# Pixel-Talk/CanonSwap

Hardware: AMD Instinct MI355X
Metric: frames/sec at 512x512 (generator hot path F->W->T->R->W->G) (higher is better)
Workload: dtype f16; 1 GPU; BASELINE configs[2]: 512x512 video, 64 frames batched per launch on each GPU, steady state over 1280 frames (20 launches per GPU) (256x256 crops in, random-init weights of the real architecture); frames_per_launch_per_gpu=64, frames_total=1280, parallelism=frame-shard x1, identities_resident=1, latency_mode=False, accumulate=fp32, debug_decodes=False

## Files before the change

### canonswap_amd/_isa.py

```python
from __future__ import annotations

import os
import subprocess

from ._build import HALO_NGROUPS, OBJ_DIR


def _disassemble(obj_dir: str, objdump: str, oname: str) -> str:
    obj = os.path.join(obj_dir, oname)
    subprocess.run([objdump, "--offloading", obj], check=True, capture_output=True)
    co = obj + ".0.hipv4-amdgcn-amd-amdhsa--gfx950"
    try:
        return subprocess.run([objdump, "-d", "--no-show-raw-insn", co], check=True, capture_output=True, text=True).stdout
    finally:
        for f in os.listdir(obj_dir):
            if f.startswith(oname + ".0."):
                os.remove(os.path.join(obj_dir, f))


def isa_check(obj_dir: str | None = None) -> dict:
    import re
    obj_dir = obj_dir or OBJ_DIR
    objdump = os.environ.get("LLVM_OBJDUMP", "/opt/rocm/lib/llvm/bin/llvm-objdump")
    if not os.path.exists(objdump):
        raise FileNotFoundError(f"isa_check: {objdump} not found")
    seen = dict(_isa_check_wide(obj_dir, objdump))
    seen.update(_isa_check_lat(obj_dir, objdump))
    for g in range(HALO_NGROUPS):
        txt = _disassemble(obj_dir, objdump, f"conv_halo_g{g}.o")
        for m in re.finditer(r"^[0-9a-f]+ <(_Z16conv_halo_kernelILi\d+ELi\d+ELi(\d+)ELi\d+ELi\d+ELi\d+ELb[01]ELb[01]ELi0EEv10ConvParams)>:\n(.*?)(?=^[0-9a-f]+ <|\Z)",
                             txt, re.S | re.M):
            name, wch, body = m.group(1), int(m.group(2)), m.group(3).split("\n")
            want = f"s_waitcnt vmcnt({3 * wch})"
            kend = max(i for i, l in enumerate(body) if "v_mfma" in l)
            waits = [i for i, l in enumerate(body) if i < kend and l.strip().startswith(want) and "lgkmcnt" not in l]
            if len(waits) < 4:
                raise RuntimeError(f"isa_check: {name}: {len(waits)} x `{want}` in the K loop, expected 4 (one per ring slot)")
            waits = waits[:4]
            loads = [(i, re.search(r"global_load_dwordx4 v\[(\d+):(\d+)\], v\[\d+:\d+\], off", l)) for i, l in enumerate(body)]
            loads = [(i, int(q.group(1))) for i, q in loads if q]
            prime = [r for i, r in loads if i < waits[0]][-4 * wch:]
            if len(prime) != 4 * wch:
                raise RuntimeError(f"isa_check: {name}: the prologue primes {len(prime)} ring registers, expected {4 * wch}")
            for k, w in enumerate(waits):
                slot = prime[k * wch:(k + 1) * wch]
                end = waits[k + 1] if k + 1 < 4 else len(body)
                seg = body[w:end]
                rel = [i for i, r in loads if w < i < end and r in slot]
                if len(rel) < wch:
                    raise RuntimeError(f"isa_check: {name}: ring slot {k} is not reloaded into v{slot} after its wait")
                first_reload = min(rel) - w
                uses = [j for j, l in enumerate(seg[:first_reload]) if "v_mfma" in l and any(f"v[{r}:{r + 3}]" in l for r in slot)]
                if not uses:
                    raise RuntimeError(f"isa_check: {name}: no MFMA reads ring slot {k} (v{slot}) between its wait and its reload")
            tail = "\n".join(body[waits[-1]:])
            if "s_waitcnt vmcnt(0)" not in tail:
                raise RuntimeError(f"isa_check: {name}: the ring is not drained (s_waitcnt vmcnt(0)) before the epilogue")
            seen[name] = len(waits)
    if not seen:
        raise RuntimeError("isa_check: no dynamic-shape conv_halo kernel found in the objects (name mangling changed?)")
    return seen


def _isa_check_lat(obj_dir: str, objdump: str) -> dict:
    import re
    txt = _disassemble(obj_dir, objdump, "conv_lat.o")
    seen = {}
    for m in re.finditer(r"^[0-9a-f]+ <(\S*conv_lat_kernel\S*)>:\n(.*?)(?=^[0-9a-f]+ <|\Z)", txt, re.S | re.M):
        name, body = m.group(1), [l.split("//")[0].strip() for l in m.group(2).split("\n")]
        body = [l for l in body if l]
        mf = [i for i, l in enumerate(body) if l.startswith("v_mfma")]
        if not mf:
            raise RuntimeError(f"isa_check: {name}: no MFMA")
        if any(l.startswith(("s_cbranch", "s_branch")) for l in body[mf[0]:mf[-1]]):
            raise RuntimeError(f"isa_check: {name}: a branch inside the K loop (the walk assumes straight-line code)")
        for i, l in enumerate(body):
            if re.search(r"\bm0\b", l):
                ok = l.startswith("s_mov_b32 m0,") and any(b.startswith("buffer_load") and b.endswith("lds") for b in body[i + 1:i + 3])
                if not ok:
                    raise RuntimeError(f"isa_check: {name}: `{l}` touches m0 outside the hidden LDS-DMA sequence")
        nvm, open_dma, nbar, ndma = 0, [], 0, 0
        for i, l in enumerate(body[:mf[-1] + 1]):
            op = l.split()[0]
            if op.startswith(("global_load", "buffer_load", "global_store", "buffer_store", "scratch_load", "scratch_store")):
                if op.startswith("buffer_load") and l.endswith("lds"):
                    open_dma.append(nvm); ndma += 1
                nvm += 1
            if op == "s_barrier":
                nbar += 1
                w = next((body[j] for j in range(i - 1, max(i - 6, -1), -1) if body[j].startswith("s_waitcnt") and "vmcnt" in body[j]), None)
                if w is None and not open_dma:
                    continue
                if w is None:
                    raise RuntimeError(f"isa_check: {name}: barrier {nbar} of the K loop has no vmcnt wait in front of it")
                n = int(re.search(r"vmcnt\((\d+)\)", w).group(1))
                for idx in open_dma:
                    if nvm - idx - 1 < n:
                        raise RuntimeError(f"isa_check: {name}: `{w}` before barrier {nbar} does not cover a DMA piece issued {nvm - idx - 1} vector-memory instructions earlier")
                open_dma = []
        if open_dma:
            raise RuntimeError(f"isa_check: {name}: {len(open_dma)} DMA pieces are never waited for at a chunk head")
        if len(mf) not in (8 * 6 * 8, 8 * 6 * 16) or ndma != 24:
            raise RuntimeError(f"isa_check: {name}: {len(mf)} MFMAs / {ndma} DMA instructions, expected 384 or 768 / 24")
        seen[name] = len(mf)
    if not seen:
        raise RuntimeError("isa_check: no conv_lat kernel found in conv_lat.o (name mangling changed?)")
    return seen


def _isa_check_wide(obj_dir: str, objdump: str) -> dict:
    seen = _isa_check_ring(obj_dir, objdump, "conv_wide.o", r"\S*conv_wide_kernel\S*", 18 * 64)
    seen.update(_isa_check_ring(obj_dir, objdump, "conv_halo_g1.o", r"_Z16conv_halo_kernelILi32ELi8ELi5ELi2ELi2ELi0ELb1ELb0ELi[789]E\S*", None))
    return seen


def _isa_check_ring(obj_dir: str, objdump: str, oname: str, name_re: str, expect_mfma) -> dict:
    import re
    txt = _disassemble(obj_dir, objdump, oname)
    seen = {}
    for m in re.finditer(r"^[0-9a-f]+ <(" + name_re + r")>:\n(.*?)(?=^[0-9a-f]+ <|\Z)", txt, re.S | re.M):
        name, body = m.group(1), m.group(2).split("\n")
        writer, waited, issued, nmfma = {}, {}, {}, 0
        pending, nvm = [], 0
        mf = [i for i, l in enumerate(body) if "v_mfma" in l]
        lo, hi = (mf[0], mf[-1]) if mf else (0, 0)
        for li, l in enumerate(body):
            t = l.split("//")[0].strip()
            if not t:
                continue
            op = t.split()[0]
            if op.startswith("s_waitcnt") and "vmcnt" in t:
                n = int(re.search(r"vmcnt\((\d+)\)", t).group(1))
                for r in waited:
                    if nvm - issued.get(r, -1) - 1 >= n:
                        waited[r] = True
                pending = [q for q in pending if nvm - q[1] - 1 < n]
            if op.startswith(("s_cbranch", "s_branch", "s_endpgm")) or li < lo:
                pending = []
            if pending and not op.startswith(("s_", "global_store", "buffer_store", "ds_write", "scratch_store")):
                mm0 = re.match(r"\S+\s+(v\[(\d+):(\d+)\]|v(\d+))", t)
                if mm0 and not (op.startswith("buffer_load") and t.endswith("lds")):
                    dst = set(range(int(mm0.group(2)), int(mm0.group(3)) + 1)) if mm0.group(2) else {int(mm0.group(4))}
                    for regs, _ in pending:
                        if regs & dst:
                            raise RuntimeError(f"isa_check: {name}: `{t}` writes v{sorted(regs & dst)} while an untracked ring load into them is in flight")
            if op.startswith(("global_load", "buffer_load", "global_store", "buffer_store", "scratch_load", "scratch_store", "global_atomic")):
                if op.startswith("global_load_dwordx4") and li >= lo:
                    q = re.match(r"\S+\s+v\[(\d+):(\d+)\]", t)
                    if q:
                        pending.append((set(range(int(q.group(1)), int(q.group(2)) + 1)), nvm))
                nvm += 1
            if op.startswith("v_mfma"):
                ops = re.findall(r"([av])\[(\d+):(\d+)\]", t)
                if len(ops) < 4 or ops[1][0] != "v":
                    raise RuntimeError(f"isa_check: {name}: MFMA with a weight operand outside the VGPRs: {t}")
                nmfma += 1
                for r in range(int(ops[1][1]), int(ops[1][2]) + 1):
                    if not writer.get(r, "").startswith("global_load_dwordx4"):
                        raise RuntimeError(f"isa_check: {name}: v{r}, a weight operand of `{t}`, was last written by `{writer.get(r)}` (a copy of a ring register?)")
                    if not waited.get(r, False):
                        raise RuntimeError(f"isa_check: {name}: no vmcnt wait between the ring load of v{r} and `{t}`")
                continue
            if op.startswith(("global_store", "buffer_store", "ds_write", "scratch_store", "s_", "buffer_load_dwordx4")) and "lds" in t + " lds" and not op.startswith("global_load"):
                if not op.startswith(("v_", "ds_read", "global_load", "scratch_load")):
                    continue
            mm = re.match(r"\S+\s+(v\[(\d+):(\d+)\]|v(\d+))", t)
            if mm and not op.startswith(("global_store", "buffer_store", "ds_write", "scratch_store")) and not (op.startswith("buffer_load") and t.endswith("lds")):
                rng = range(int(mm.group(2)), int(mm.group(3)) + 1) if mm.group(2) else [int(mm.group(4))]
                is_vm = op.startswith(("global_load", "buffer_load", "scratch_load"))
                for r in rng:
                    writer[r] = op
                    waited[r] = False
                    issued[r] = (nvm - 1) if is_vm else -1
        if expect_mfma is not None and nmfma != expect_mfma:
            raise RuntimeError(f"isa_check: {name}: {nmfma} MFMAs in the kernel, expected {expect_mfma}")
        seen[name] = nmfma
    if not seen:
        raise RuntimeError(f"isa_check: no kernel matching {name_re} found in {oname} (name mangling changed?)")
    return seen
```

### canonswap_amd/csrc/vol32.hip

```cpp
#include "conv_epilogue.h"

namespace {

constexpr int V_TW = 8;
constexpr int V_NC = V_TW + 2;
constexpr int V_CS = 17 * 16;
constexpr int V_RS = V_NC * V_CS;
constexpr int V_WLO = 27 * 2 * 1024;
constexpr int V_SROWS = 8;
enum { V_EPI_F16 = 0,
       V_EPI_RES = 1,
       V_EPI_STAT = 2 };

template <bool SPLIT, int EPI = 0> struct VRing {
    static constexpr int K = SPLIT ? 2 : 4;
    static constexpr int RING = K + 2;
    static constexpr int QS = ((RING * V_RS + 16 + 255) / 256) * 256;
    static constexpr int IMG = 4 * QS;
    static constexpr int NIMG = SPLIT ? 2 : 1;
    static constexpr int AUX = NIMG * IMG;
    static constexpr int RROWS = K + 1;
    static constexpr int RSLOT = 4 * 4096;
    static constexpr int lds(int epi) { return AUX + (SPLIT ? V_WLO : 0) + (epi == 1 ? RROWS * RSLOT : 0); }
};

struct Vol32Params {
    const half_t* in; const half_t* zero;
    int in_sN, in_sH, in_sW;
    int N, H, W;
    const half_t* wgt;
    const float* bias;
    float sl0, sl1;
    const float* res; int res_sN, res_sH, res_sW;
    void* out0; int o0_sN, o0_sH, o0_sW;
    half_t* out1; int o1_sN, o1_sH, o1_sW;
    const float* s2; const float* t2;
    float* stat_out; int stat_nblk;
    int srows;
    const float* xf_y; int xy_sN, xy_sH, xy_sW;
    const float* xf_res; int xr_sN, xr_sH, xr_sW;
    float* xf_out; int xo_sN, xo_sH, xo_sW;
    const float* xf_stats; const float* xf_gamma; const float* xf_beta; float xf_slope;
    int nstrips, nseg, seg_rows, items;
#ifdef V32_TL
    unsigned long long* tl; long tl_cap;
#endif
};

typedef unsigned int u4v __attribute__((ext_vector_type(4)));

#ifdef V32_TL
#define TLS(i) do { __builtin_amdgcn_sched_barrier(0); const unsigned long long t_ = __builtin_amdgcn_s_memtime(); tl_acc[i] += t_ - tl_last; tl_last = t_; \
                    __builtin_amdgcn_sched_barrier(0); } while (0)
#else
#define TLS(i) do { } while (0)
#endif

template <int N> __device__ __forceinline__ void wait_vm() { asm volatile("s_waitcnt vmcnt(%0)" ::"n"(N) : "memory"); }

template <int EPI, bool SPLIT, int XF>
__global__ void __launch_bounds__(256, 1) vol32_kernel(const Vol32Params p)
{
    static_assert(XF == 0 || (SPLIT && EPI == V_EPI_STAT), "transform staging exists for the split-precision statistics kernel");
    extern __shared__ __attribute__((aligned(16))) unsigned char smem[];
    using R = VRing<SPLIT, EPI>;
    constexpr int K = R::K, RING = R::RING, QS = R::QS, IMG = R::IMG, NIMG = R::NIMG;
    constexpr int VOX = SPLIT ? 64 : 32;
    static_assert(!(SPLIT && EPI == V_EPI_RES), "the residual ring and the W_lo fragments share the LDS region after the images");
    constexpr int ND = XF ? 0 : 3 * NIMG + (EPI == V_EPI_RES ? 4 : 0), NR = 0, NS = EPI == V_EPI_F16 ? 2 : (EPI == V_EPI_RES ? 6 : 4);
    constexpr int NW0 = NR + (K - 2) * (ND + NR + NS), NW = NW0 + NS;
    static_assert(NW <= 63, "vmcnt is a 6-bit counter");
    const int tid = threadIdx.x, lane = tid & 63;
    const int wave = __builtin_amdgcn_readfirstlane(tid >> 6);
    const int l15 = lane & 15, l4 = lane >> 4;
#ifdef V32_TL
    unsigned long long tl_acc[10] = {0, 0, 0, 0, 0, 0, 0, 0, 0, 0}, tl_last = __builtin_amdgcn_s_memtime();
#endif

    for (int i = tid * 16; i < NIMG * IMG; i += 256 * 16) *(u4v*)(smem + i) = (u4v){0u, 0u, 0u, 0u};
    h8_t wr[27][2];
    {
        const half_t* wl = p.wgt + ep_lane_row(1, l15) * 32 + l4 * 8;
#pragma unroll
        for (int t = 0; t < 27; ++t) {
            wr[t][0] = *(const h8_t*)(wl + t * 1024 + ep_frag_row(1, 0) * 32);
            wr[t][1] = *(const h8_t*)(wl + t * 1024 + ep_frag_row(1, 1) * 32);
        }
        if constexpr (SPLIT) {
            for (int f = wave; f < 54; f += 4) {
                const h8_t v = *(const h8_t*)(wl + (27 + (f >> 1)) * 1024 + ep_frag_row(1, f & 1) * 32);
                *(h8_t*)(smem + R::AUX + f * 1024 + lane * 16) = v;
            }
        }
    }
    float bias_v[8], s2_v[8], t2_v[8];
#pragma unroll
    for (int r = 0; r < 8; ++r) {
        bias_v[r] = p.bias ? p.bias[l4 * 8 + r] : 0.f;
        s2_v[r] = p.s2 ? p.s2[l4 * 8 + r] : 1.f;
        t2_v[r] = p.s2 ? p.t2[l4 * 8 + r] : 0.f;
    }
    __syncthreads();

    int s_off[3]; bool s_on[3];
#pragma unroll
    for (int j = 0; j < 3; ++j) {
        const int idx = j * 64 + lane, col = idx / 17, ds = idx % 17;
        s_on[j] = idx < V_NC * 17 && ds != 0;
        s_off[j] = col * p.in_sW + (ds - 1) * VOX + wave * 8;
    }
    const int lanebase = l4 * QS + l15 * 16 + (2 * wave) * V_CS;
    const unsigned lane_el = (unsigned)(l15 * 32 + l4 * 8);
    const unsigned char* wlo = smem + R::AUX + lane * 16;

    const int G = (int)gridDim.x;
    int u = (int)blockIdx.x;
    if ((G & 7) == 0) u = (u & 7) * (G >> 3) + (u >> 3);

    for (int item = u; item < p.items; item += G) {
        int t = item;
        const int strip = t % p.nstrips; t /= p.nstrips;
        const int seg = t % p.nseg;
        const int n = t / p.nseg;
        const int w0 = strip * V_TW;
        const int h0 = seg * p.seg_rows, h1 = (h0 + p.seg_rows < p.H) ? h0 + p.seg_rows : p.H;
        bool c_ok[3];
#pragma unroll
        for (int j = 0; j < 3; ++j) {
            const int col = (j * 64 + lane) / 17;
            c_ok[j] = s_on[j] && (unsigned)(w0 - 1 + col) < (unsigned)p.W;
        }
        const half_t* in_n = p.in + (long)n * p.in_sN + (long)(w0 - 1) * p.in_sW;
        const unsigned nb_o0 = (unsigned)(n * p.o0_sN + (w0 + 2 * wave) * p.o0_sW);
        const unsigned nb_o1 = (unsigned)(n * p.o1_sN + (w0 + 2 * wave) * p.o1_sW);
        const unsigned nb_rs = (unsigned)(n * p.res_sN + (w0 + 2 * wave) * p.res_sW);
        auto stage_piece = [&](int r, int slot, int rslot, int q) {
            if (q < 3 * NIMG) {
                const int im = q / 3, j = q % 3;
                const bool rok = (unsigned)r < (unsigned)p.H && r <= h1;
                const half_t* rp = in_n + (long)r * p.in_sH;
                unsigned char* dst = smem + wave * QS + slot * V_RS;
                if (s_on[j]) {
                    const half_t* src = (rok && c_ok[j]) ? rp + s_off[j] + im * 32 : p.zero;
                    __builtin_amdgcn_global_load_lds((const __attribute__((address_space(1))) void*)src,
                                                     (__attribute__((address_space(3))) void*)(dst + im * IMG + j * 1024), 16, 0, 0);
                }
            } else if constexpr (EPI == V_EPI_RES) {
                const int j = q - 3 * NIMG;
                const int rc = (unsigned)r < (unsigned)p.H ? r : 0;
                const float* rsrc = p.res + (nb_rs + (unsigned)(rc * p.res_sH) + lane_el);
                unsigned char* rdst = smem + R::AUX + rslot * R::RSLOT + wave * 4096;
                __builtin_amdgcn_global_load_lds((const __attribute__((address_space(1))) void*)(rsrc + (j >> 1) * p.res_sW + (j & 1) * 4),
                                                 (__attribute__((address_space(3))) void*)(rdst + j * 1024), 16, 0, 0);
            }
        };
        auto stage_row = [&](int r, int slot, int rslot) {
#pragma unroll
            for (int q = 0; q < ND; ++q) stage_piece(r, slot, rslot, q);
        };
        constexpr bool XRES = XF >= 2 && ((XF - 2) & 1) != 0, XWB = XF >= 2 && ((XF - 2) & 2) != 0;
        float4 xr[XF ? 3 : 1][2], xs[XRES ? 3 : 1][2];
        float xsc[XF >= 2 ? 8 : 1], xsh[XF >= 2 ? 8 : 1];
        const int xq = tid & 3;
        if constexpr (XF >= 2) {
#pragma unroll
            for (int r = 0; r < 8; ++r) {
                const int c = xq * 8 + r;
                const float mean = p.xf_stats[((long)n * 32 + c) * 2], rstd = p.xf_stats[((long)n * 32 + c) * 2 + 1];
                xsc[r] = gn_scale(rstd, p.xf_gamma[c]);
                xsh[r] = gn_shift(mean, xsc[r], p.xf_beta[c]);
            }
        }
        int xoff[XF ? 3 : 1]; bool xcok[XF ? 3 : 1];
        if constexpr (XF != 0) {
#pragma unroll
            for (int it = 0; it < 3; ++it) {
                int idx = it * 256 + tid;
                if (idx >= V_NC * 64) idx -= 128;
                const int col = idx >> 6, d = (idx >> 2) & 15;
                xoff[it] = n * p.xy_sN + (w0 - 1 + col) * p.xy_sW + d * 32 + xq * 8;
                xcok[it] = (unsigned)(w0 - 1 + col) < (unsigned)p.W;
            }
        }
        const unsigned xsafe = (unsigned)(n * p.xy_sN + w0 * p.xy_sW + h0 * p.xy_sH + ((tid >> 2) & 15) * 32 + xq * 8);
        auto xf_load_to = [&](int r, int it, float4 (&dr)[2], float4 (&ds)[2]) {
            if constexpr (XF != 0) {
                const bool okl = xcok[it] && (unsigned)r < (unsigned)p.H && r <= h1;
                const unsigned o = okl ? (unsigned)(xoff[it] + r * p.xy_sH) : xsafe;
                const float* y = p.xf_y + o;
                dr[0] = *(const float4*)y; dr[1] = *(const float4*)(y + 4);
                if constexpr (XRES) {
                    const float* x = p.xf_res + o;
                    ds[0] = *(const float4*)x; ds[1] = *(const float4*)(x + 4);
                }
            }
        };
        auto xf_load = [&](int r, int it) { xf_load_to(r, it, xr[it], xs[XRES ? it : 0]); };
        float xa[8];
        auto xf_write_from = [&](int r, int slot, int it, int part, const float4 (&xr)[2], const float4 (&xs)[2]) {
            if constexpr (XF != 0) {
                int idx = it * 256 + tid;
                if (idx >= V_NC * 64) idx -= 128;
                const bool ok = xcok[it] && (unsigned)r < (unsigned)p.H && r <= h1;
#pragma unroll
                for (int k = 0; k < 8; ++k) {
                    if (part >= 0 && (k >> 2) != part) continue;
                    const float v = ((const float*)&xr[k >> 2])[k & 3];
                    if constexpr (XRES) xa[k] = gn_lrelu(v, xsc[k], xsh[k], ((const float*)&xs[k >> 2])[k & 3], p.xf_slope);
                    else if constexpr (XF >= 2) xa[k] = gn_lrelu(v, xsc[k], xsh[k], 0.f, p.xf_slope);
                    else xa[k] = v;
                    if (!ok) xa[k] = 0.f;
                }
                if (part >= 0 && part != 2) return;
                h8_t hi, lo;
#pragma unroll
                for (int k = 0; k < 8; ++k) { hi[k] = (half_t)xa[k]; lo[k] = (half_t)(xa[k] - (float)hi[k]); }
                unsigned char* dst = smem + xq * QS + (idx >> 6) * V_CS + (((idx >> 2) & 15) + 1) * 16 + slot * V_RS;
                *(h8_t*)dst = hi; *(h8_t*)(dst + IMG) = lo;
                if constexpr (XWB) {
                    float* o = ok ? p.xf_out + (unsigned)(xoff[it] + r * p.xy_sH) : (float*)p.zero;
                    *(float4*)o = make_float4(xa[0], xa[1], xa[2], xa[3]); *(float4*)(o + 4) = make_float4(xa[4], xa[5], xa[6], xa[7]);
                }
            }
        };
        auto xf_write = [&](int r, int slot, int it, int part) { xf_write_from(r, slot, it, part, xr[it], xs[XRES ? it : 0]); };
        if constexpr (XF != 0) {
            float4 pr[3][3][2], ps[XRES ? 3 : 1][3][2];
#pragma unroll
            for (int i = 0; i < 3; ++i)
#pragma unroll
                for (int it = 0; it < 3; ++it) xf_load_to(h0 - 1 + i, it, pr[i][it], ps[XRES ? i : 0][it]);
#pragma unroll
            for (int i = 0; i < 3; ++i)
#pragma unroll
                for (int it = 0; it < 3; ++it) xf_write_from(h0 - 1 + i, i, it, -1, pr[i][it], ps[XRES ? i : 0][it]);
        } else {
#pragma unroll
            for (int i = 0; i <= K; ++i) stage_row(h0 - 1 + i, i, i == 0 ? K : i - 1);
        }
        TLS(0);
        __syncthreads();
        TLS(1);

        float ov[2][8]; h8_t ou[2];
        bool have = false;
        int hprev = 0;
        auto store_piece = [&](int k) {
            constexpr int PC = NS / 2;
            const int c = k / PC, w = k % PC;
            const unsigned o = nb_o0 + (unsigned)(hprev * p.o0_sH + c * p.o0_sW) + lane_el;
            if constexpr (EPI != V_EPI_F16) {
                if (w == 0) *(float4*)((float*)p.out0 + o) = make_float4(ov[c][0], ov[c][1], ov[c][2], ov[c][3]);
                if (w == 1) *(float4*)((float*)p.out0 + o + 4) = make_float4(ov[c][4], ov[c][5], ov[c][6], ov[c][7]);
                if constexpr (EPI == V_EPI_RES) {
                    if (w == 2) *(h8_t*)(p.out1 + (nb_o1 + (unsigned)(hprev * p.o1_sH + c * p.o1_sW) + lane_el)) = ou[c];
                }
            } else {
                h8_t x;
#pragma unroll
                for (int r = 0; r < 8; ++r) x[r] = ep_h(ov[c][r]);
                *(h8_t*)((half_t*)p.out0 + o) = x;
            }
        };
        auto flush = [&]() {
#pragma unroll
            for (int k = 0; k < NS; ++k) store_piece(k);
        };
        float st_s[8], st_q[8];
#pragma unroll
        for (int r = 0; r < 8; ++r) { st_s[r] = 0.f; st_q[r] = 0.f; }

        int s0 = 0, r0 = 0;
        for (int h = h0; h < h1; ++h) {
            int sk = s0 + K + 1; sk -= sk >= RING ? RING : 0;
            int rk = r0 + K; rk -= rk >= R::RROWS ? R::RROWS : 0;
            f4_t rr[2][2];
            if constexpr (EPI == V_EPI_RES) {
#pragma unroll
                for (int c = 0; c < 2; ++c)
#pragma unroll
                    for (int i = 0; i < 2; ++i) rr[c][i] = *(const f4_t*)(wlo + r0 * R::RSLOT + wave * 4096 + (c * 2 + i) * 1024);
            }
            int rb[3];
#pragma unroll
            for (int kh = 0; kh < 3; ++kh) { int sl = s0 + kh; sl -= sl >= RING ? RING : 0; rb[kh] = lanebase + sl * V_RS; }
            f4_t acc[2][2];
#pragma unroll
            for (int c = 0; c < 2; ++c)
#pragma unroll
                for (int ci = 0; ci < 2; ++ci) acc[c][ci] = (f4_t){0.f, 0.f, 0.f, 0.f};
            constexpr int NG = SPLIT ? 27 : 9;
            constexpr int XL0 = 4, XW0 = 17;
            h8_t fa[4], fb[4];
            h8_t wa[SPLIT ? 3 : 1][2], wb[SPLIT ? 3 : 1][2];
            auto rd = [&](h8_t (&f)[4], h8_t (&wl2)[SPLIT ? 3 : 1][2], int G2) {
                const int pass = G2 / 9, g = G2 % 9, kd = g / 3, kh = g % 3;
                const int img = (SPLIT && pass == 2) ? IMG : 0;
#pragma unroll
                for (int i = 0; i < 4; ++i) f[i] = *(const h8_t*)(smem + rb[kh] + img + i * V_CS + kd * 16);
                if constexpr (SPLIT) {
                    if (pass == 1) {
#pragma unroll
                        for (int kw = 0; kw < 3; ++kw)
#pragma unroll
                            for (int ci = 0; ci < 2; ++ci) wl2[kw][ci] = *(const h8_t*)(wlo + ((g * 3 + kw) * 2 + ci) * 1024);
                    }
                }
            };
            rd(fa, wa, 0);
#pragma unroll
            for (int G2 = 0; G2 < NG; ++G2) {
                h8_t (&cur)[4] = (G2 & 1) ? fb : fa;
                h8_t (&wcur)[SPLIT ? 3 : 1][2] = (G2 & 1) ? wb : wa;
                h8_t (&wnxt)[SPLIT ? 3 : 1][2] = (G2 & 1) ? wa : wb;
                if constexpr (XF != 0) { if (G2 >= XW0 && G2 < XW0 + 9) xf_write(h + 2, sk, (G2 - XW0) / 3, (G2 - XW0) % 3); }
                if (G2 + 1 < NG) {
                    h8_t (&nxt)[4] = (G2 & 1) ? fa : fb;
                    rd(nxt, wnxt, G2 + 1);
                }
                const int pass = G2 / 9, g = G2 % 9;
#pragma unroll
                for (int kw = 0; kw < 3; ++kw)
#pragma unroll
                    for (int c = 0; c < 2; ++c)
#pragma unroll
                        for (int ci = 0; ci < 2; ++ci) {
                            const h8_t a = (SPLIT && pass == 1) ? wcur[SPLIT ? kw : 0][ci] : wr[g * 3 + kw][ci];
                            acc[c][ci] = __builtin_amdgcn_mfma_f32_16x16x32_f16(a, cur[kw + c], acc[c][ci], 0, 0, 0);
                        }
                if (G2 + 1 < NG) {
                    const int nrd = 4 + ((SPLIT && (G2 + 1) / 9 == 1) ? 6 : 0);
                    const bool conv_here = XF != 0 && G2 >= XW0 && G2 < XW0 + 9;
#pragma unroll
                    for (int i = 0; i < 11; ++i) {
                        __builtin_amdgcn_sched_group_barrier(0x008, 1, 0);
                        if (i < nrd) __builtin_amdgcn_sched_group_barrier(0x100, 1, 0);
                        if (conv_here) __builtin_amdgcn_sched_group_barrier(0x002, 4, 0);
                    }
                }
                __builtin_amdgcn_sched_barrier(0);
                if constexpr (XF == 0) {
                    constexpr int NM = ND + NS;
#pragma unroll
                    for (int m = G2 * NM / NG; m < (G2 + 1) * NM / NG; ++m) {
                        asm volatile("" ::: "memory");
                        if (m < ND) stage_piece(h + K, sk, rk, m);
                        else if (have) store_piece(m - ND);
                        asm volatile("" ::: "memory");
                    }
                    __builtin_amdgcn_sched_barrier(0);
                } else {
                    if (G2 < NS && have) store_piece(G2);
                    if (G2 >= XL0 && G2 < XL0 + 6 && ((G2 - XL0) & 1) == 0) xf_load(h + 2, (G2 - XL0) >> 1);
                    __builtin_amdgcn_sched_barrier(0);
                }
            }
            TLS(4);
#pragma unroll
            for (int c = 0; c < 2; ++c) {
#pragma unroll
                for (int r = 0; r < 8; ++r) {
                    float v = acc[c][r >> 2][r & 3] + bias_v[r];
                    v = lin_act(v, p.sl0);
                    if constexpr (EPI == V_EPI_RES) v += rr[c][r >> 2][r & 3];
                    ov[c][r] = v;
                    if constexpr (EPI == V_EPI_STAT) { st_s[r] += v; st_q[r] = fmaf(v, v, st_q[r]); }
                    if constexpr (EPI == V_EPI_RES) {
                        const float a = v * s2_v[r] + t2_v[r];
                        ou[c][r] = ep_h(lin_act(a, p.sl1));
                    }
                }
            }
            if constexpr (EPI == V_EPI_STAT) {
                if (((h + 1) % p.srows) == 0 || h + 1 == h1) {
                    const int blk = (h / p.srows) * (p.W / 2) + (w0 / 2 + wave);
                    float pa[8], pb[8];
#pragma unroll
                    for (int r = 0; r < 8; ++r) {
                        float a = st_s[r], b = st_q[r];
                        st_s[r] = 0.f; st_q[r] = 0.f;
#pragma unroll
                        for (int o = 1; o < 16; o <<= 1) { a += __shfl_xor(a, o, 64); b += __shfl_xor(b, o, 64); }
                        pa[r] = a; pb[r] = b;
                    }
                    if (l15 == 0) {
                        float4* dst = (float4*)(p.stat_out + (((long)n * p.stat_nblk + blk) * 32 + l4 * 8) * 2);
#pragma unroll
                        for (int r = 0; r < 4; ++r) dst[r] = make_float4(pa[2 * r], pb[2 * r], pa[2 * r + 1], pb[2 * r + 1]);
                    }
                }
            }
            have = true; hprev = h;
            s0 = s0 + 1 == RING ? 0 : s0 + 1;
            r0 = r0 + 1 == R::RROWS ? 0 : r0 + 1;
            TLS(5);
            if constexpr (XF != 0) asm volatile("s_waitcnt lgkmcnt(0)" ::: "memory");
            else if (h > h0 + K - 2) wait_vm<NW>();
            else wait_vm<NW0>();
            TLS(6);
            __builtin_amdgcn_s_barrier();
            asm volatile("" ::: "memory");
            TLS(7);
#ifdef V32_TL
            tl_acc[9] += 1;
#endif
        }
        if (have) flush();
        __syncthreads();
        TLS(8);
    }
#ifdef V32_TL
    if (p.tl && lane == 0) {
        const long wi = (long)blockIdx.x * 4 + wave;
        if (wi < p.tl_cap) {
            unsigned hwid;
            asm volatile("s_getreg_b32 %0, hwreg(HW_REG_HW_ID)" : "=s"(hwid));
            unsigned long long* o = p.tl + wi * 12;
#pragma unroll
            for (int i = 0; i < 10; ++i) o[i] = tl_acc[i];
            o[10] = hwid; o[11] = __builtin_amdgcn_s_memrealtime();
        }
    }
#endif
}

int g_ncu = 0;
#ifdef V32_TL
unsigned long long* g_v32_tl = nullptr;
long g_v32_cap = 0;
#endif

}

#ifdef V32_TL
extern "C" void cs_debug_set_vol32_tl(void* buf, long cap) { g_v32_tl = (unsigned long long*)buf; g_v32_cap = cap; }
#endif

bool vol32_supported(const ConvParams& p)
{
    if (p.KD != 3 || p.KH != 3 || p.KW != 3 || p.Cout_pad != 32 || p.Cout != 32 || p.D != 16 || p.inD != 16 || (p.W % V_TW) != 0) return false;
    if (p.xf_kind) {
        if (!p.hilo || p.Cin != 96 || !p.stat_out || (p.xf_kind != 1 && p.xf_kind != 2) || !p.xf_y.p || p.xf_y.sD != 32) return false;
        if (p.xf_kind == 2 && (!p.xf_stats || !p.xf_gamma || !p.xf_beta)) return false;
        if (p.xf_res.p && (p.xf_kind != 2 || p.xf_res.sD != 32)) return false;
        if (p.xf_out.p && (p.xf_kind != 2 || p.xf_out.sD != 32)) return false;
    } else if (p.hilo ? (p.Cin != 96 || p.in_sD != 64) : (p.Cin != 32 || p.in_sD != 32)) return false;
    if (p.up_shift || p.cg || p.wslot || p.sk_out || p.ragged || p.pixscale || p.stats || p.pool_hw || p.spmul) return false;
    if (p.act0 > ACT_LRELU || p.act1 > ACT_LRELU) return false;
    if (p.res.p && (!p.res_f32 || p.res.sD != 32)) return false;
    if (p.out0.p && p.out0.sD != 32) return false;
    if (p.out1.p && p.out1.sD != 32) return false;
    if (!p.out0.p) return false;
    if (p.hilo && !p.stat_out) return false;
    if (p.stat_out) return p.out0_f32 && !p.res.p && !p.out1.p;
    if (p.res.p) return p.out0_f32 && p.out1.p && !p.hilo;
    return !p.out0_f32 && !p.out1.p;
}

static int vol32_srows(const ConvParams& p) { return p.v32_srows > 0 ? p.v32_srows : V_SROWS; }
int vol32_stat_nblk(const ConvParams& p) { const int sr = vol32_srows(p); return ((p.H + sr - 1) / sr) * (p.W / 2); }

int launch_vol32(const ConvParams& p, hipStream_t st)
{
    if (!vol32_supported(p)) { cs_set_error("vol32: not a 3x3x3 32 -> 32 convolution on a [N][H][W][16][32] volume this kernel supports"); return -1; }
    if (ep_check_extents(p, "vol32")) return -1;
    const long in_span = (long)(p.N - 1) * p.in_sN + (long)(p.H - 1) * p.in_sH + (long)(p.W - 1) * p.in_sW + 1024;
    if (!p.xf_kind && in_span >= (1L << 31)) { cs_set_error("vol32: the input spans 2^31 elements or more"); return -1; }
    if (!g_ncu) {
        int dev = 0, n = 0;
        if (hipGetDevice(&dev) != hipSuccess || hipDeviceGetAttribute(&n, hipDeviceAttributeMultiprocessorCount, dev) != hipSuccess || n < 1) n = 256;
        g_ncu = n;
    }
    Vol32Params k;
    k.in = p.in; k.zero = p.zero; k.in_sN = (int)p.in_sN; k.in_sH = (int)p.in_sH; k.in_sW = (int)p.in_sW;
    k.N = p.N; k.H = p.H; k.W = p.W;
    k.wgt = p.wgt; k.bias = p.bias;
    k.sl0 = p.act0 == ACT_NONE ? 1.f : (p.act0 == ACT_LRELU ? p.slope0 : 0.f);
    k.sl1 = p.act1 == ACT_NONE ? 1.f : (p.act1 == ACT_LRELU ? p.slope1 : 0.f);
    k.res = (const float*)p.res.p; k.res_sN = (int)p.res.sN; k.res_sH = (int)p.res.sH; k.res_sW = (int)p.res.sW;
    k.out0 = p.out0.p; k.o0_sN = (int)p.out0.sN; k.o0_sH = (int)p.out0.sH; k.o0_sW = (int)p.out0.sW;
    k.out1 = (half_t*)p.out1.p; k.o1_sN = (int)p.out1.sN; k.o1_sH = (int)p.out1.sH; k.o1_sW = (int)p.out1.sW;
    k.s2 = p.s2; k.t2 = p.t2;
    k.stat_out = p.stat_out; k.stat_nblk = vol32_stat_nblk(p); k.srows = vol32_srows(p);
    k.xf_y = (const float*)p.xf_y.p; k.xy_sN = (int)p.xf_y.sN; k.xy_sH = (int)p.xf_y.sH; k.xy_sW = (int)p.xf_y.sW;
    k.xf_res = (const float*)p.xf_res.p; k.xr_sN = (int)p.xf_res.sN; k.xr_sH = (int)p.xf_res.sH; k.xr_sW = (int)p.xf_res.sW;
    k.xf_out = (float*)p.xf_out.p; k.xo_sN = (int)p.xf_out.sN; k.xo_sH = (int)p.xf_out.sH; k.xo_sW = (int)p.xf_out.sW;
    k.xf_stats = p.xf_stats; k.xf_gamma = p.xf_gamma; k.xf_beta = p.xf_beta; k.xf_slope = p.xf_slope;
    if (p.xf_kind) {
        auto same = [&](const TDesc& t) { return !t.p || (t.sN == p.xf_y.sN && t.sH == p.xf_y.sH && t.sW == p.xf_y.sW); };
        if (!same(p.xf_res) || !same(p.xf_out)) { cs_set_error("vol32: the transform-staging volumes must share their strides"); return -1; }
        const long lim = 1L << 31;
        auto span = [&](const TDesc& t) { return (long)(p.N - 1) * t.sN + (long)(p.H - 1) * t.sH + (long)(p.W - 1) * t.sW + 512; };
        if (span(p.xf_y) >= lim || (p.xf_res.p && span(p.xf_res) >= lim) || (p.xf_out.p && span(p.xf_out) >= lim)) {
            cs_set_error("vol32: a transform-staging tensor spans 2^31 elements or more"); return -1;
        }
    }
#ifdef V32_TL
    k.tl = g_v32_tl; k.tl_cap = g_v32_cap;
#endif
    k.nstrips = p.W / V_TW;
    int nseg = 1;
    while ((long)p.N * k.nstrips * nseg < g_ncu && (p.H % (nseg * 2 * k.srows)) == 0) nseg *= 2;
    k.seg_rows = (p.H + nseg - 1) / nseg;
    k.nseg = (p.H + k.seg_rows - 1) / k.seg_rows;
    k.items = p.N * k.nstrips * k.nseg;
    int grid = k.items < g_ncu ? k.items : g_ncu;
    if (grid >= 8) grid &= ~7;
    const bool split = p.hilo != 0;
    const int epi = p.stat_out ? V_EPI_STAT : (p.res.p ? V_EPI_RES : V_EPI_F16);
    auto go = [&](auto kern, size_t lds) -> int {
        if (lds > 64 * 1024) {
            hipError_t e = hipFuncSetAttribute((const void*)kern, hipFuncAttributeMaxDynamicSharedMemorySize, (int)lds);
            if (e != hipSuccess) { cs_set_error("vol32: opting into %zu bytes of LDS failed: %s", lds, hipGetErrorString(e)); return -1; }
        }
        hipLaunchKernelGGL(kern, dim3((unsigned)grid), dim3(256), lds, st, k);
        return 0;
    };
    int r = -1;
    if (split) {
        if (epi != V_EPI_STAT) { cs_set_error("vol32: the split-precision kernel exists with the statistics epilogue only"); return -1; }
        if (p.xf_kind == 2) {
            const int v = (p.xf_res.p ? 1 : 0) | (p.xf_out.p ? 2 : 0);
            if (v == 0) r = go(vol32_kernel<V_EPI_STAT, true, 2>, VRing<true, V_EPI_STAT>::lds(V_EPI_STAT));
            else if (v == 1) r = go(vol32_kernel<V_EPI_STAT, true, 3>, VRing<true, V_EPI_STAT>::lds(V_EPI_STAT));
            else if (v == 2) r = go(vol32_kernel<V_EPI_STAT, true, 4>, VRing<true, V_EPI_STAT>::lds(V_EPI_STAT));
            else r = go(vol32_kernel<V_EPI_STAT, true, 5>, VRing<true, V_EPI_STAT>::lds(V_EPI_STAT));
        }
        else if (p.xf_kind == 1) r = go(vol32_kernel<V_EPI_STAT, true, 1>, VRing<true, V_EPI_STAT>::lds(V_EPI_STAT));
        else r = go(vol32_kernel<V_EPI_STAT, true, 0>, VRing<true, V_EPI_STAT>::lds(V_EPI_STAT));
    } else {
        if (epi == V_EPI_STAT) r = go(vol32_kernel<V_EPI_STAT, false, 0>, VRing<false, V_EPI_STAT>::lds(V_EPI_STAT));
        else if (epi == V_EPI_RES) r = go(vol32_kernel<V_EPI_RES, false, 0>, VRing<false, V_EPI_RES>::lds(V_EPI_RES));
        else r = go(vol32_kernel<V_EPI_F16, false, 0>, VRing<false, V_EPI_F16>::lds(V_EPI_F16));
    }
    if (r) return r;
    hipError_t e = hipGetLastError();
    if (e != hipSuccess) { cs_set_error("vol32 launch: %s", hipGetErrorString(e)); return -1; }
    return 0;
}
```

Measured before the change: 536.3 frames/s.

## Add eight-wave vol32 kernel splitting output channels across wave pairs

Adds a 512-thread variant of the split-precision vol32 3D conv kernel for the transform-staging cases. Each pair of waves splits the 32 output channels into two 16-channel fragments, so a wave holds only its half of the weights in registers. The staging loads and transforms for row h+2 are interleaved into the MFMA loop with sched_group_barriers. It is on by default behind an env var and is verified by a new ISA check for MFMA count, no scratch or AGPR use, and correct waitcnt placement. The trade-off is more waves per block at launch bounds of one block per CU, with the intent of better latency hiding, at the cost of more barrier participants.

```diff
diff --git a/canonswap_amd/_isa.py b/canonswap_amd/_isa.py
--- a/canonswap_amd/_isa.py
+++ b/canonswap_amd/_isa.py
@@ -26,6 +26,7 @@
         raise FileNotFoundError(f"isa_check: {objdump} not found")
     seen = dict(_isa_check_wide(obj_dir, objdump))
     seen.update(_isa_check_lat(obj_dir, objdump))
+    seen.update(_isa_check_vol32_w8(obj_dir, objdump))
     for g in range(HALO_NGROUPS):
         txt = _disassemble(obj_dir, objdump, f"conv_halo_g{g}.o")
         for m in re.finditer(r"^[0-9a-f]+ <(_Z16conv_halo_kernelILi\d+ELi\d+ELi(\d+)ELi\d+ELi\d+ELi\d+ELb[01]ELb[01]ELi0EEv10ConvParams)>:\n(.*?)(?=^[0-9a-f]+ <|\Z)",
@@ -105,6 +106,42 @@
         seen[name] = len(mf)
     if not seen:
         raise RuntimeError("isa_check: no conv_lat kernel found in conv_lat.o (name mangling changed?)")
+    return seen
+
+
+def _isa_check_vol32_w8(obj_dir: str, objdump: str) -> dict:
+    import re
+    txt = _disassemble(obj_dir, objdump, "vol32.o")
+    seen = {}
+    for m in re.finditer(r"^[0-9a-f]+ <(\S*vol32_w8_kernelILi(\d)E\S*)>:\n(.*?)(?=^[0-9a-f]+ <|\Z)", txt, re.S | re.M):
+        name, body = m.group(1), [l.split("//")[0].strip() for l in m.group(3).split("\n")]
+        body = [l for l in body if l]
+        mf = [i for i, l in enumerate(body) if l.startswith("v_mfma")]
+        if len(mf) != 162:
+            raise RuntimeError(f"isa_check: {name}: {len(mf)} MFMAs, expected 162")
+        top = max((i for i, l in enumerate(body[:mf[0]]) if l == "s_barrier"), default=0)
+        since = None
+        for l in body[top:mf[-1] + 1]:
+            op = l.split()[0]
+            if op.startswith("global_load"):
+                since = 0
+            elif op.startswith(("global_store", "global_atomic")) and since is not None:
+                since += 1
+            elif op == "s_waitcnt" and "vmcnt" in l:
+                n = int(re.search(r"vmcnt\((\d+)\)", l).group(1))
+                if since is None or n < since:
+                    raise RuntimeError(f"isa_check: {name}: `{l}` in the K loop waits for more than the staging loads in front of it "
+                                       "(a load result carried over the back-edge?)")
+        for l in body:
+            if l.startswith("scratch_") or re.search(r"\ba(\d+|\[\d+:\d+\])", l):
+                raise RuntimeError(f"isa_check: {name}: `{l}`: scratch or AGPRs in a kernel with a 256-register budget")
+        tail = body[mf[-1]:]
+        bar = next((i for i, l in enumerate(tail) if l == "s_barrier"), None)
+        if bar is None or not any(l.startswith("s_waitcnt") and "lgkmcnt(0)" in l for l in tail[max(bar - 4, 0):bar]):
+            raise RuntimeError(f"isa_check: {name}: no `s_waitcnt lgkmcnt(0)` in front of the step's barrier")
+        seen[name] = len(mf)
+    if sorted(int(re.search(r"vol32_w8_kernelILi(\d)E", k).group(1)) for k in seen) != [1, 2, 3, 5]:
+        raise RuntimeError(f"isa_check: vol32.o holds the eight-wave instantiations {sorted(seen)}, expected XF 1, 2, 3, 5")
     return seen
 
 
diff --git a/canonswap_amd/csrc/vol32.hip b/canonswap_amd/csrc/vol32.hip
--- a/canonswap_amd/csrc/vol32.hip
+++ b/canonswap_amd/csrc/vol32.hip
@@ -412,6 +412,254 @@
 #ifdef V32_TL
     if (p.tl && lane == 0) {
         const long wi = (long)blockIdx.x * 4 + wave;
+        if (wi < p.tl_cap) {
+            unsigned hwid;
+            asm volatile("s_getreg_b32 %0, hwreg(HW_REG_HW_ID)" : "=s"(hwid));
+            unsigned long long* o = p.tl + wi * 12;
+#pragma unroll
+            for (int i = 0; i < 10; ++i) o[i] = tl_acc[i];
+            o[10] = hwid; o[11] = __builtin_amdgcn_s_memrealtime();
+        }
+    }
+#endif
+}
+
+template <int XF>
+__global__ void __launch_bounds__(512, 1) vol32_w8_kernel(const Vol32Params p)
+{
+    static_assert(XF >= 1 && XF <= 5, "the eight-wave form exists for the transform-staging variants");
+    extern __shared__ __attribute__((aligned(16))) unsigned char smem[];
+    using R = VRing<true, V_EPI_STAT>;
+    constexpr int K = R::K, RING = R::RING, QS = R::QS, IMG = R::IMG;
+    static_assert(K == 2, "row h + 2 is fetched, transformed and written within step h");
+    constexpr int NS = 2;
+    constexpr int NP = V_NC * 128;
+    const int tid = threadIdx.x, lane = tid & 63;
+    const int wave = __builtin_amdgcn_readfirstlane(tid >> 6);
+    const int cp = wave & 3, fr = wave >> 2;
+    const int l15 = lane & 15, l4 = lane >> 4;
+#ifdef V32_TL
+    unsigned long long tl_acc[10] = {0, 0, 0, 0, 0, 0, 0, 0, 0, 0}, tl_last = __builtin_amdgcn_s_memtime();
+#endif
+
+    for (int i = tid * 16; i < 2 * IMG; i += 512 * 16) *(u4v*)(smem + i) = (u4v){0u, 0u, 0u, 0u};
+    h8_t wr[27];
+    {
+        const half_t* wl = p.wgt + (fr * 16 + l15) * 32 + l4 * 8;
+#pragma unroll
+        for (int t = 0; t < 27; ++t) wr[t] = *(const h8_t*)(wl + t * 1024);
+        for (int t = cp; t < 27; t += 4) {
+            const h8_t v = *(const h8_t*)(wl + (27 + t) * 1024);
+            *(h8_t*)(smem + R::AUX + (t * 2 + fr) * 1024 + lane * 16) = v;
+        }
+    }
+    float bias_v[4];
+#pragma unroll
+    for (int r = 0; r < 4; ++r) bias_v[r] = p.bias ? p.bias[fr * 16 + l4 * 4 + r] : 0.f;
+    __syncthreads();
+
+    const int lanebase = l4 * QS + l15 * 16 + (2 * cp) * V_CS;
+    const unsigned lane_el = (unsigned)(l15 * 32 + fr * 16 + l4 * 4);
+    const unsigned char* wlo = smem + R::AUX + fr * 1024 + lane * 16;
+
+    const int G = (int)gridDim.x;
+    int u = (int)blockIdx.x;
+    if ((G & 7) == 0) u = (u & 7) * (G >> 3) + (u >> 3);
+
+    for (int item = u; item < p.items; item += G) {
+        int t = item;
+        const int strip = t % p.nstrips; t /= p.nstrips;
+        const int seg = t % p.nseg;
+        const int n = t / p.nseg;
+        const int w0 = strip * V_TW;
+        const int h0 = seg * p.seg_rows, h1 = (h0 + p.seg_rows < p.H) ? h0 + p.seg_rows : p.H;
+        const unsigned nb_o0 = (unsigned)(n * p.o0_sN + (w0 + 2 * cp) * p.o0_sW);
+        constexpr bool XRES = XF >= 2 && ((XF - 2) & 1) != 0, XWB = XF >= 2 && ((XF - 2) & 2) != 0;
+        float4 xr[3], xs[XRES ? 3 : 1];
+        float xsc[XF >= 2 ? 4 : 1], xsh[XF >= 2 ? 4 : 1];
+        const int xc = tid & 7;
+        if constexpr (XF >= 2) {
+#pragma unroll
+            for (int r = 0; r < 4; ++r) {
+                const int c = xc * 4 + r;
+                const float mean = p.xf_stats[((long)n * 32 + c) * 2], rstd = p.xf_stats[((long)n * 32 + c) * 2 + 1];
+                xsc[r] = gn_scale(rstd, p.xf_gamma[c]);
+                xsh[r] = gn_shift(mean, xsc[r], p.xf_beta[c]);
+            }
+        }
+        auto xf_idx = [&](int it) { const int idx = it * 512 + tid; return idx >= NP ? idx - 256 : idx; };
+        int xoff[3]; bool xcok[3];
+#pragma unroll
+        for (int it = 0; it < 3; ++it) {
+            const int idx = xf_idx(it), col = idx >> 7, d = (idx >> 3) & 15;
+            xoff[it] = n * p.xy_sN + (w0 - 1 + col) * p.xy_sW + d * 32 + xc * 4;
+            xcok[it] = (unsigned)(w0 - 1 + col) < (unsigned)p.W;
+        }
+        const unsigned xsafe = (unsigned)(n * p.xy_sN + w0 * p.xy_sW + h0 * p.xy_sH + ((tid >> 3) & 15) * 32 + xc * 4);
+        auto xf_load_to = [&](int r, int it, float4& dr, float4& ds) {
+            const bool okl = xcok[it] && (unsigned)r < (unsigned)p.H && r <= h1;
+            const unsigned o = okl ? (unsigned)(xoff[it] + r * p.xy_sH) : xsafe;
+            dr = *(const float4*)(p.xf_y + o);
+            if constexpr (XRES) ds = *(const float4*)(p.xf_res + o);
+        };
+        auto xf_load = [&](int r, int it) { xf_load_to(r, it, xr[it], xs[XRES ? it : 0]); };
+        float xa[4];
+        auto xf_write_from = [&](int r, int slot, int it, int part, const float4& yr, const float4& sr) {
+            const int idx = xf_idx(it);
+            const bool ok = xcok[it] && (unsigned)r < (unsigned)p.H && r <= h1;
+            if (part <= 0) {
+#pragma unroll
+                for (int k = 0; k < 4; ++k) {
+                    const float v = ((const float*)&yr)[k];
+                    if constexpr (XRES) xa[k] = gn_lrelu(v, xsc[k], xsh[k], ((const float*)&sr)[k], p.xf_slope);
+                    else if constexpr (XF >= 2) xa[k] = gn_lrelu(v, xsc[k], xsh[k], 0.f, p.xf_slope);
+                    else xa[k] = v;
+                    if (!ok) xa[k] = 0.f;
+                }
+            }
+            if (part == 0) return;
+            h4_t hi, lo;
+#pragma unroll
+            for (int k = 0; k < 4; ++k) { hi[k] = (half_t)xa[k]; lo[k] = (half_t)(xa[k] - (float)hi[k]); }
+            unsigned char* dst = smem + (xc >> 1) * QS + (idx >> 7) * V_CS + (((idx >> 3) & 15) + 1) * 16 + (xc & 1) * 8 + slot * V_RS;
+            *(h4_t*)dst = hi; *(h4_t*)(dst + IMG) = lo;
+            if constexpr (XWB) {
+                float* o = ok ? p.xf_out + (unsigned)(xoff[it] + r * p.xy_sH) : (float*)p.zero;
+                *(float4*)o = make_float4(xa[0], xa[1], xa[2], xa[3]);
+            }
+        };
+        auto xf_write = [&](int r, int slot, int it, int part) { xf_write_from(r, slot, it, part, xr[it], xs[XRES ? it : 0]); };
+        {
+            float4 pr[3][3], ps[XRES ? 3 : 1][3];
+#pragma unroll
+            for (int i = 0; i < 3; ++i)
+#pragma unroll
+                for (int it = 0; it < 3; ++it) xf_load_to(h0 - 1 + i, it, pr[i][it], ps[XRES ? i : 0][it]);
+#pragma unroll
+            for (int i = 0; i < 3; ++i)
+#pragma unroll
+                for (int it = 0; it < 3; ++it) xf_write_from(h0 - 1 + i, i, it, -1, pr[i][it], ps[XRES ? i : 0][it]);
+        }
+        TLS(0);
+        __syncthreads();
+        TLS(1);
+
+        float ov[2][4];
+        bool have = false;
+        int hprev = 0;
+        auto store_piece = [&](int c) {
+            const unsigned o = nb_o0 + (unsigned)(hprev * p.o0_sH + c * p.o0_sW) + lane_el;
+            *(float4*)((float*)p.out0 + o) = make_float4(ov[c][0], ov[c][1], ov[c][2], ov[c][3]);
+        };
+        float st_s[4], st_q[4];
+#pragma unroll
+        for (int r = 0; r < 4; ++r) { st_s[r] = 0.f; st_q[r] = 0.f; }
+
+        int s0 = 0;
+        for (int h = h0; h < h1; ++h) {
+            int sk = s0 + K + 1; sk -= sk >= RING ? RING : 0;
+            int rb[3];
+#pragma unroll
+            for (int kh = 0; kh < 3; ++kh) { int sl = s0 + kh; sl -= sl >= RING ? RING : 0; rb[kh] = lanebase + sl * V_RS; }
+            f4_t acc[2];
+#pragma unroll
+            for (int c = 0; c < 2; ++c) acc[c] = (f4_t){0.f, 0.f, 0.f, 0.f};
+            constexpr int NG = 27;
+            constexpr int XL0 = 4, XW0 = 17;
+            h8_t fa[4], fb[4];
+            h8_t wa[3], wb[3];
+            auto rd = [&](h8_t (&f)[4], h8_t (&wl2)[3], int G2) {
+                const int pass = G2 / 9, g = G2 % 9, kd = g / 3, kh = g % 3;
+                const int img = pass == 2 ? IMG : 0;
+#pragma unroll
+                for (int i = 0; i < 4; ++i) f[i] = *(const h8_t*)(smem + rb[kh] + img + i * V_CS + kd * 16);
+                if (pass == 1) {
+#pragma unroll
+                    for (int kw = 0; kw < 3; ++kw) wl2[kw] = *(const h8_t*)(wlo + ((g * 3 + kw) * 2) * 1024);
+                }
+            };
+            rd(fa, wa, 0);
+#pragma unroll
+            for (int G2 = 0; G2 < NG; ++G2) {
+                h8_t (&cur)[4] = (G2 & 1) ? fb : fa;
+                h8_t (&wcur)[3] = (G2 & 1) ? wb : wa;
+                h8_t (&wnxt)[3] = (G2 & 1) ? wa : wb;
+                const bool conv_here = G2 >= XW0 && G2 < XW0 + 6;
+                if (conv_here) xf_write(h + 2, sk, (G2 - XW0) / 2, (G2 - XW0) % 2);
+                if (G2 + 1 < NG) {
+                    h8_t (&nxt)[4] = (G2 & 1) ? fa : fb;
+                    rd(nxt, wnxt, G2 + 1);
+                }
+                const int pass = G2 / 9, g = G2 % 9;
+#pragma unroll
+                for (int kw = 0; kw < 3; ++kw)
+#pragma unroll
+                    for (int c = 0; c < 2; ++c) {
+                        const h8_t a = pass == 1 ? wcur[kw] : wr[g * 3 + kw];
+                        acc[c] = __builtin_amdgcn_mfma_f32_16x16x32_f16(a, cur[kw + c], acc[c], 0, 0, 0);
+                    }
+                if (G2 + 1 < NG) {
+                    const int nrd = 4 + ((G2 + 1) / 9 == 1 ? 3 : 0);
+#pragma unroll
+                    for (int i = 0; i < 5; ++i) {
+                        __builtin_amdgcn_sched_group_barrier(0x008, 1, 0);
+                        if (i < nrd) __builtin_amdgcn_sched_group_barrier(0x100, 1, 0);
+                        if (i + 5 < nrd) __builtin_amdgcn_sched_group_barrier(0x100, 1, 0);
+                        if (conv_here) __builtin_amdgcn_sched_group_barrier(0x002, 6, 0);
+                    }
+                }
+                __builtin_amdgcn_sched_barrier(0);
+                if (G2 < NS && have) store_piece(G2);
+                if (G2 >= XL0 && G2 < XL0 + 6 && ((G2 - XL0) & 1) == 0) xf_load(h + 2, (G2 - XL0) >> 1);
+                __builtin_amdgcn_sched_barrier(0);
+            }
+            TLS(4);
+#pragma unroll
+            for (int c = 0; c < 2; ++c) {
+#pragma unroll
+                for (int r = 0; r < 4; ++r) {
+                    float v = acc[c][r] + bias_v[r];
+                    v = lin_act(v, p.sl0);
+                    ov[c][r] = v;
+                    st_s[r] += v; st_q[r] = fmaf(v, v, st_q[r]);
+                }
+            }
+            if (((h + 1) % p.srows) == 0 || h + 1 == h1) {
+                const int blk = (h / p.srows) * (p.W / 2) + (w0 / 2 + cp);
+                float pa[4], pb[4];
+#pragma unroll
+                for (int r = 0; r < 4; ++r) {
+                    pa[r] = ep_row_sum16(st_s[r]); pb[r] = ep_row_sum16(st_q[r]);
+                    st_s[r] = 0.f; st_q[r] = 0.f;
+                }
+                if (l15 == 0) {
+                    float4* dst = (float4*)(p.stat_out + (((long)n * p.stat_nblk + blk) * 32 + fr * 16 + l4 * 4) * 2);
+                    dst[0] = make_float4(pa[0], pb[0], pa[1], pb[1]);
+                    dst[1] = make_float4(pa[2], pb[2], pa[3], pb[3]);
+                }
+            }
+            have = true; hprev = h;
+            s0 = s0 + 1 == RING ? 0 : s0 + 1;
+            TLS(5);
+            asm volatile("s_waitcnt lgkmcnt(0)" ::: "memory");
+            TLS(6);
+            __builtin_amdgcn_s_barrier();
+            asm volatile("" ::: "memory");
+            TLS(7);
+#ifdef V32_TL
+            tl_acc[9] += 1;
+#endif
+        }
+        if (have) {
+#pragma unroll
+            for (int c = 0; c < NS; ++c) store_piece(c);
+        }
+        __syncthreads();
+        TLS(8);
+    }
+#ifdef V32_TL
+    if (p.tl && lane == 0) {
+        const long wi = (long)blockIdx.x * 8 + wave;
         if (wi < p.tl_cap) {
             unsigned hwid;
             asm volatile("s_getreg_b32 %0, hwreg(HW_REG_HW_ID)" : "=s"(hwid));
@@ -508,18 +756,29 @@
     if (grid >= 8) grid &= ~7;
     const bool split = p.hilo != 0;
     const int epi = p.stat_out ? V_EPI_STAT : (p.res.p ? V_EPI_RES : V_EPI_F16);
+    int threads = 256;
     auto go = [&](auto kern, size_t lds) -> int {
         if (lds > 64 * 1024) {
             hipError_t e = hipFuncSetAttribute((const void*)kern, hipFuncAttributeMaxDynamicSharedMemorySize, (int)lds);
             if (e != hipSuccess) { cs_set_error("vol32: opting into %zu bytes of LDS failed: %s", lds, hipGetErrorString(e)); return -1; }
         }
-        hipLaunchKernelGGL(kern, dim3((unsigned)grid), dim3(256), lds, st, k);
+        hipLaunchKernelGGL(kern, dim3((unsigned)grid), dim3(threads), lds, st, k);
         return 0;
     };
     int r = -1;
     if (split) {
         if (epi != V_EPI_STAT) { cs_set_error("vol32: the split-precision kernel exists with the statistics epilogue only"); return -1; }
-        if (p.xf_kind == 2) {
+        static const bool w8_on = [] { const char* s = getenv("CANONSWAP_VOL32_W8"); return !s || atoi(s) != 0; }();
+        const int xfv = p.xf_kind == 2 ? 2 + ((p.xf_res.p ? 1 : 0) | (p.xf_out.p ? 2 : 0)) : p.xf_kind;
+        if (w8_on && p.v32_srows <= 0 && xfv != 0 && xfv != 4) {
+            threads = 512;
+            const size_t lds = VRing<true, V_EPI_STAT>::lds(V_EPI_STAT);
+            if (xfv == 1) r = go(vol32_w8_kernel<1>, lds);
+            else if (xfv == 2) r = go(vol32_w8_kernel<2>, lds);
+            else if (xfv == 3) r = go(vol32_w8_kernel<3>, lds);
+            else r = go(vol32_w8_kernel<5>, lds);
+        }
+        else if (p.xf_kind == 2) {
             const int v = (p.xf_res.p ? 1 : 0) | (p.xf_out.p ? 2 : 0);
             if (v == 0) r = go(vol32_kernel<V_EPI_STAT, true, 2>, VRing<true, V_EPI_STAT>::lds(V_EPI_STAT));
             else if (v == 1) r = go(vol32_kernel<V_EPI_STAT, true, 3>, VRing<true, V_EPI_STAT>::lds(V_EPI_STAT));
```

Result: no change. 539.5 frames/s, median of 6 (+0.6%).
